# magicat777/Audio-Analyzer-OMEGA

Measured on NVIDIA B200. Metric: stream-seconds of 48 kHz stereo analysed/sec (multi-res FFT+LUFS+TP), higher is better.
Workload: dtype f32 (FFT, combine, K-weighting in a float32 delta-form state, sample peaks of the true-peak meter; its four transforms per frame pair in f16x2; tensor-core GEMM on (hi, lo) half operands with fp32 accumulators for the few-bin resolutions) + f64 (meter statistics)

## Files before the change

### audio-analyzer-omega_b200/csrc/omega4_cuda.cu

```cuda
#include "../../include/omega4_cuda.h"

#include <cuda_runtime.h>
#include <math.h>
#include <stdio.h>
#include <stdlib.h>
#include <string.h>

#include <algorithm>
#include <map>
#include <mutex>
#include <set>
#include <string>
#include <vector>

#include "bars_kernel.cuh"
#include "blockdft_kernel.cuh"
#include "blockdft_tc_kernel.cuh"
#include "fft_core.cuh"
#include "kweight_kernel.cuh"
#include "kweight32_kernel.cuh"
#include "loudness_kernel.cuh"
#include "misc_kernels.cuh"
#include "octave_kernel.cuh"
#include "multires_kernel.cuh"
// ... 22 lines not shown
    } while (0)

extern "C" const char* omega4_last_error(void) { return g_err.c_str(); }
extern "C" int omega4_abi_version(void) { return OMEGA4_ABI_VERSION; }
extern "C" int omega4_device_count(void) {
    int n = 0;
    if (cudaGetDeviceCount(&n) != cudaSuccess) { cudaGetLastError(); return 0; }
    return n;
}

static int ilog2(int n) { int l = 0; while ((1 << l) < n) ++l; return l; }
static bool is_pow2(int n) { return n > 0 && (n & (n - 1)) == 0; }

struct Twiddles { float2* twM = nullptr; float2* twN = nullptr; float2* tw4W = nullptr; };
static std::mutex g_tw_mu;
static std::map<std::pair<int, int>, Twiddles> g_tw;

static int get_twiddles(int device, int log2m, Twiddles* out) {
    std::lock_guard<std::mutex> lk(g_tw_mu);
    auto key = std::make_pair(device, log2m);
    auto it = g_tw.find(key);
    if (it != g_tw.end()) { *out = it->second; return OMEGA4_OK; }
    const int M = 1 << log2m, N = 2 * M;
    const double two_pi = 6.283185307179586476925287;
    std::vector<float2> a(M), b(M / 2 + 1), c(3 * M + 1);
    for (int e = 0; e < M; ++e) a[e] = make_float2((float)cos(two_pi * e / M), (float)-sin(two_pi * e / M));
    for (int k = 0; k <= M / 2; ++k) b[k] = make_float2((float)cos(two_pi * k / N), (float)-sin(two_pi * k / N));
    for (int j = 0; j <= 3 * M; ++j) c[j] = make_float2((float)cos(two_pi * j / (4.0 * N)), (float)sin(two_pi * j / (4.0 * N)));
    Twiddles t;
    CK(cudaMalloc(&t.twM, a.size() * sizeof(float2)));
    CK(cudaMalloc(&t.twN, b.size() * sizeof(float2)));
    CK(cudaMalloc(&t.tw4W, c.size() * sizeof(float2)));
    CK(cudaMemcpy(t.twM, a.data(), a.size() * sizeof(float2), cudaMemcpyHostToDevice));
    CK(cudaMemcpy(t.twN, b.data(), b.size() * sizeof(float2), cudaMemcpyHostToDevice));
    CK(cudaMemcpy(t.tw4W, c.data(), c.size() * sizeof(float2), cudaMemcpyHostToDevice));
    g_tw[key] = t;
    *out = t;
    return OMEGA4_OK;
}

template <int L>
static int launch_multires_t(const MultiresArgs& a, cudaStream_t s) {
    using S = FftShape<L>;
    const int fpc = a.rounds * S::CONC;
    const long long tiles = (a.n_frames + fpc - 1) / fpc;
    const long long grid = tiles * a.n_ch;
    if (grid <= 0) return OMEGA4_OK;
    if (grid > 2147483647LL) return fail(OMEGA4_ERR_INVALID, "multires grid too large");
    if constexpr (L <= 12) {
        const size_t smem = multires_local_smem_bytes<L>(a.need_cnt, a.n_tb);
        CK(cudaFuncSetAttribute(multires_local_kernel<L>, cudaFuncAttributeMaxDynamicSharedMemorySize, (int)smem));
        multires_local_kernel<L><<<(unsigned)grid, 256, smem, s>>>(a);
    } else {
        const size_t smem = multires_smem_bytes<L>(a.need_cnt);
        CK(cudaFuncSetAttribute(multires_kernel<L>, cudaFuncAttributeMaxDynamicSharedMemorySize, (int)smem));
        multires_kernel<L><<<(unsigned)grid, S::NT, smem, s>>>(a);
    }
    CK(cudaGetLastError());
    return OMEGA4_OK;
}

static int launch_multires(int log2m, const MultiresArgs& a, cudaStream_t s) {
    switch (log2m) {
        case 8: return launch_multires_t<8>(a, s);
        case 9: return launch_multires_t<9>(a, s);
        case 10: return launch_multires_t<10>(a, s);
        case 11: return launch_multires_t<11>(a, s);
        case 12: return launch_multires_t<12>(a, s);
        case 13: return launch_multires_t<13>(a, s);
        case 14: return launch_multires_t<14>(a, s);
    }
    return fail(OMEGA4_ERR_UNSUPPORTED, "fft size must be a power of two in 512 .. 32768");
}

static int default_rounds(int n_frames, int conc) {
    int r = 16;
    while (r > 1 && (long long)r * conc > n_frames) r >>= 1;
    return r;
}

static void fill_truepeak_steps(TruePeakArgs* t) {
    const double two_pi = 6.283185307179586476925287;
    for (int p = 1; p <= 3; ++p) {
        for (int j = 0; j < 16; ++j) {
            const int jj = j < 8 ? j : j - 16;
            t->step[p - 1][j] = make_float2((float)cos(two_pi * p * jj / 64.0), (float)sin(two_pi * p * jj / 64.0));
        }
        t->nyq[p - 1] = (float)cos(two_pi * p / 8.0);
    }
}

static int launch_truepeak(const TruePeakArgs& a, cudaStream_t s) {
    constexpr int L = 11;
    using S = FftShape<L>;
    const size_t smem = truepeak_smem_bytes<L>();
    CK(cudaFuncSetAttribute(truepeak_kernel<L>, cudaFuncAttributeMaxDynamicSharedMemorySize, (int)smem));
    const int ppc = a.rounds * S::CONC;
    const int n_pairs = (a.n_frames + 1) / 2;
    const long long grid = (long long)((n_pairs + ppc - 1) / ppc) * a.n_ch;
    if (grid <= 0) return OMEGA4_OK;
    if (grid > 2147483647LL) return fail(OMEGA4_ERR_INVALID, "truepeak grid too large");
    truepeak_kernel<L><<<(unsigned)grid, S::NT, smem, s>>>(a);
    CK(cudaGetLastError());
    return OMEGA4_OK;
}

static int launch_truepeak16(const TruePeakArgs& a, cudaStream_t s) {
    constexpr int L = 11;
    using S = FftShape<L>;
    const size_t smem = truepeak16_smem_bytes<L>();
    CK(cudaFuncSetAttribute(truepeak16_kernel<L>, cudaFuncAttributeMaxDynamicSharedMemorySize, (int)smem));
    const int ppc = a.rounds * S::CONC;
    const int n_pairs = (a.n_frames + 1) / 2;
    const long long grid = (long long)((n_pairs + ppc - 1) / ppc) * a.n_ch;
    if (grid <= 0) return OMEGA4_OK;
    if (grid > 2147483647LL) return fail(OMEGA4_ERR_INVALID, "truepeak grid too large");
    truepeak16_kernel<L><<<(unsigned)grid, S::NT, smem, s>>>(a);
    CK(cudaGetLastError());
    return OMEGA4_OK;
}

template <bool F64, bool WT>
static int launch_kweight_t(const KweightArgs& a, cudaStream_t s) {
    const size_t smem = kweight_smem_bytes();
    CK(cudaFuncSetAttribute(kweight_kernel<F64, WT>, cudaFuncAttributeMaxDynamicSharedMemorySize, (int)smem));
    const int fpc = a.frames_per_warp * KW_WARPS;
    const long long grid = (long long)((a.n_frames + fpc - 1) / fpc) * a.n_ch;
    if (grid <= 0) return OMEGA4_OK;
    if (grid > 2147483647LL) return fail(OMEGA4_ERR_INVALID, "kweight grid too large");
    kweight_kernel<F64, WT><<<(unsigned)grid, KW_WARPS * 32, smem, s>>>(a);
    CK(cudaGetLastError());
    return OMEGA4_OK;
}

static int launch_kweight(const KweightArgs& a, cudaStream_t s) {
    if (a.x_is_f64) return a.weighted_out ? launch_kweight_t<true, true>(a, s) : launch_kweight_t<true, false>(a, s);
    return a.weighted_out ? launch_kweight_t<false, true>(a, s) : launch_kweight_t<false, false>(a, s);
}

static int launch_kweight32(const Kweight32Args& a, cudaStream_t s) {
    const size_t smem = kweight32_smem_bytes();
    CK(cudaFuncSetAttribute(kweight32_kernel, cudaFuncAttributeMaxDynamicSharedMemorySize, (int)smem));
    const int fpc = a.frames_per_warp * KW32_WARPS;
    const long long grid = (long long)((a.n_frames + fpc - 1) / fpc) * a.n_ch;
    if (grid <= 0) return OMEGA4_OK;
    if (grid > 2147483647LL) return fail(OMEGA4_ERR_INVALID, "kweight grid too large");
    kweight32_kernel<<<(unsigned)grid, KW32_WARPS * 32, smem, s>>>(a);
    CK(cudaGetLastError());
    return OMEGA4_OK;
}

static int launch_stats(const StatsArgs& a, cudaStream_t s) {
    if (a.n_ch <= 0) return OMEGA4_OK;
    if (!a.fresh && a.n_frames == 1 && a.first_frame == 0 && !getenv("OMEGA4_STATS_WALK")) {
        stats_push1_kernel<<<a.n_ch, ST_P1_THREADS, 0, s>>>(a);
    } else if (a.fresh) {
        const size_t smem = stats_smem_bytes<false>();
        CK(cudaFuncSetAttribute(stats_kernel<false>, cudaFuncAttributeMaxDynamicSharedMemorySize, (int)smem));
        stats_kernel<false><<<a.n_ch, ST_THREADS, smem, s>>>(a);
    } else {
        const size_t smem = stats_smem_bytes<true>();
        CK(cudaFuncSetAttribute(stats_kernel<true>, cudaFuncAttributeMaxDynamicSharedMemorySize, (int)smem));
        stats_kernel<true><<<a.n_ch, ST_THREADS, smem, s>>>(a);
    }
    CK(cudaGetLastError());
    return OMEGA4_OK;
}

static int launch_s16_convert(const int16_t* in, long long stream_stride, int il, int n_streams, long long n_frames,
                              float* out, long long out_stride, cudaStream_t s) {
    if (n_streams <= 0 || n_frames <= 0) return OMEGA4_OK;
    if (n_streams > 65535) return fail(OMEGA4_ERR_INVALID, "too many streams for one int16 conversion launch (max 65535)");
    const long long per_stream = n_frames * il;
    dim3 grid((unsigned)((per_stream + 1023) / 1024), (unsigned)n_streams);
    s16_deinterleave_kernel<<<grid, 256, 0, s>>>(in, stream_stride, il, n_frames, out, out_stride);
    CK(cudaGetLastError());
    return OMEGA4_OK;
}

static void mat2_mul(const double* a, const double* b, double* c) {
    double r[4] = {a[0] * b[0] + a[1] * b[2], a[0] * b[1] + a[1] * b[3],
                   a[2] * b[0] + a[3] * b[2], a[2] * b[1] + a[3] * b[3]};
    memcpy(c, r, sizeof r);
}

static void build_biquad(const double* b, const double* a, int order, KwBiquad* q) {
    memset(q, 0, sizeof *q);
    const double a0 = a[0];
    q->b0 = b[0] / a0; q->b1 = b[1] / a0; q->b2 = order >= 2 ? b[2] / a0 : 0.0;
    q->a1 = a[1] / a0; q->a2 = order >= 2 ? a[2] / a0 : 0.0;
    q->pad = 3 * (order + 1);
    if (order >= 2) {
        double zi0, zi1;
        const double m00 = 1.0 + q->a1, m01 = -1.0, m10 = q->a2, m11 = 1.0;
        const double r0 = q->b1 - q->a1 * q->b0, r1 = q->b2 - q->a2 * q->b0;
        const double det = m00 * m11 - m01 * m10;
        zi0 = (r0 * m11 - m01 * r1) / det;
        zi1 = (m00 * r1 - m10 * r0) / det;
        q->yi0 = -zi1 / q->a2;
        q->yi1 = (-zi0 + q->a1 * zi1 / q->a2) / q->a2;
    } else {
        const double zi0 = (q->b1 - q->a1 * q->b0) / (1.0 + q->a1);
        q->yi0 = -zi0 / q->a1;
        q->yi1 = 0.0;
    }
    const double Cm[4] = {-q->a1, -q->a2, 1.0, 0.0};
    double P[4] = {Cm[0], Cm[1], Cm[2], Cm[3]};
    for (int i = 0; i < KW_L; ++i) {
        if (i < KW_SUBMAX) { q->g[i][0] = P[0]; q->g[i][1] = P[1]; }
        if (i + 1 == 16) memcpy(q->c16, P, sizeof P);
        if (i + 1 == 17) memcpy(q->c17, P, sizeof P);
        if (i + 1 < KW_L) mat2_mul(Cm, P, P);
    }
    memcpy(q->phi[0], P, sizeof P);
    for (int j = 1; j < 5; ++j) mat2_mul(q->phi[j - 1], q->phi[j - 1], q->phi[j]);
    auto inv_pow = [&](int k, double* out) {
        if (k == 0) { out[0] = 1; out[1] = 0; out[2] = 0; out[3] = 1; return; }
        if (order >= 2) {
            const double det1 = Cm[0] * Cm[3] - Cm[1] * Cm[2];
            const double Ci[4] = {Cm[3] / det1, -Cm[1] / det1, -Cm[2] / det1, Cm[0] / det1};
            double R[4] = {Ci[0], Ci[1], Ci[2], Ci[3]};
            for (int i = 1; i < k; ++i) mat2_mul(Ci, R, R);
            memcpy(out, R, sizeof R);
        } else {
            out[0] = pow(-q->a1, -(double)k); out[1] = 0; out[2] = 0; out[3] = 0;
        }
    };
    inv_pow(KW_PAD - q->pad, q->cinv_f);
    inv_pow(KW_SLACK + KW_PAD - q->pad, q->cinv_b);
}

struct ResInfo {
    int n = 0, log2m = 0, bins = 0;
    float weight = 1.f;
    float* window = nullptr;
    float* binw = nullptr;
    int n_tb = 0;
    int* tb_idx = nullptr;
    int* tb_lo = nullptr;
    float* tb_frac = nullptr;
    int need_lo = 0, need_cnt = 0;
    Twiddles tw;
};

struct SparseRes {
    int r = 0, nk = 0, nt = 0, B = 0, col0 = 0;
    bool td = false;
    int xoff = 0;
    float2* T = nullptr;
    float* kw = nullptr;
    int* tb_pos = nullptr;
};

struct SparseSet {
    int n = 0;
    SparseRes sp[OMEGA4_MAX_RES];
    int of_res[OMEGA4_MAX_RES];
    int cols = 0, qs = 0;
    float* E = nullptr;
    uint8_t* Eimg = nullptr;
    float e_inv = 1.f;
    int n_halves = 0;
    bool fusable = false;
    int nkx = 0;
    short gB[TC_MAX_GROUPS], gX[TC_MAX_GROUPS], gN[TC_MAX_GROUPS], gS[TC_MAX_GROUPS];
    SparseSet() { for (int i = 0; i < OMEGA4_MAX_RES; ++i) of_res[i] = -1; }
    void release() {
        for (int i = 0; i < OMEGA4_MAX_RES; ++i) { cudaFree(sp[i].T); cudaFree(sp[i].kw); cudaFree(sp[i].tb_pos); }
        cudaFree(E); cudaFree(Eimg);
    }
};

struct DevBuf {
    void* p = nullptr;
    size_t cap = 0;
    int ensure(size_t bytes) {
        if (bytes <= cap) return OMEGA4_OK;
        if (p) cudaFree(p);
        p = nullptr; cap = 0;
        CK(cudaMalloc(&p, bytes));
        cap = bytes;
        return OMEGA4_OK;
    }
    void release() { if (p) cudaFree(p); p = nullptr; cap = 0; }
};

struct omega4_bars {
    int device = 0, T = 0, n_valid = 0, p_lo = 0, normalize_max = 0;
    float p_frac = 0.f, scale = 0.8f;
    int* bands = nullptr; float* gain = nullptr; float* sf = nullptr; float* sfc = nullptr;
    DevBuf h_spec, h_out, h_peak, h_state, state_in;
};

static int bars_launch(omega4_bars* b, cudaStream_t s, const float* spec, int n_ch, int n_hops, float* state, int fresh,
                       float* band_values, float* peak_values, DevBuf* state_copy) {
    BarsArgs a;
    memset(&a, 0, sizeof a);
    a.T = b->T; a.n_ch = n_ch; a.n_hops = n_hops; a.n_valid = b->n_valid; a.bands = b->bands; a.gain = b->gain;
    a.sf = b->sf; a.sfc = b->sfc; a.p_lo = b->p_lo; a.p_frac = b->p_frac; a.scale = b->scale;
    a.normalize_max = b->normalize_max; a.fresh = (fresh || !state) ? 1 : 0;
    a.spec = spec; a.bars_out = band_values; a.peaks_out = peak_values; a.state = state;
    const size_t st_bytes = (size_t)n_ch * (1 + b->n_valid) * sizeof(float);
    const size_t smem = bars_smem_bytes(b->T, b->n_valid);
    if (smem > 200 * 1024) return fail(OMEGA4_ERR_UNSUPPORTED, "spectrum too long for the bars kernel");
    if (b->T > 32 * BARS_MAXV) return fail(OMEGA4_ERR_UNSUPPORTED, "spectrum too long for the bars kernel (max 1024 bins)");
    if (b->T <= 512) CK(cudaFuncSetAttribute(bars_kernel<16>, cudaFuncAttributeMaxDynamicSharedMemorySize, (int)smem));
    else CK(cudaFuncSetAttribute(bars_kernel<32>, cudaFuncAttributeMaxDynamicSharedMemorySize, (int)smem));
    a.seg = n_ch >= 1024 ? 4 * BARS_SEG : BARS_SEG;
    const long long grid = (long long)n_ch * ((n_hops + a.seg - 1) / a.seg);
    if (grid > 2147483647LL) return fail(OMEGA4_ERR_INVALID, "bars grid too large");
    if (a.state && !a.fresh && n_hops > a.seg) {
        int rc = state_copy->ensure(st_bytes); if (rc) return rc;
        CK(cudaMemcpyAsync(state_copy->p, a.state, st_bytes, cudaMemcpyDeviceToDevice, s));
        a.state_in = (const float*)state_copy->p;
    }
    if (b->T <= 512) bars_kernel<16><<<(unsigned)grid, BARS_WARPS * 32, smem, s>>>(a);
// ... 1970 lines not shown
```

### audio-analyzer-omega_b200/csrc/stats_kernel.cuh

```cuda
#pragma once
#include <cuda_runtime.h>
#include <math_constants.h>

namespace o4 {

constexpr int ST_M = 24;
constexpr int ST_S = 180;
constexpr int ST_I = 3600;
constexpr int ST_P = 60;
constexpr int ST_SORT = 4096;
constexpr int ST_THREADS = 32;
constexpr int ST_STATE = 8 + ST_I + ST_P;

struct StatsArgs {
    const double* lufs;
    const double* tp;
    int n_ch;
    int n_frames;
    int first_frame;
    double gate;
    double* state;
    float* out;
    int fresh;
};

__device__ __forceinline__ double st_percentile(const double* s, int n, double q) {
    double vi = (double)n * q + (1.0 + q * (1.0 - 1.0 - 1.0)) - 1.0;
    if (vi < 0.0) vi = 0.0;
    if (vi > (double)(n - 1)) vi = (double)(n - 1);
    double fl = floor(vi);
    int lo = (int)fl;
    int hi = lo + 1 < n ? lo + 1 : n - 1;
    double t = vi - fl;
    double av = s[lo], bv = s[hi];
    double d = bv - av;
    return (t >= 0.5) ? (bv - d * (1.0 - t)) : (av + d * t);
}

__device__ __forceinline__ int warp_lower_bound(const float* s, int n, float v, int lane) {
    int lo = 0, hi = n;
    while (lo < hi) {
        const int step = (hi - lo + 31) >> 5;
        const int idx = lo + lane * step;
        const bool less = (idx < hi) && (s[idx] < v);
        const int c = __popc(__ballot_sync(0xffffffffu, less));
        if (step == 1) return lo + c;
        if (c == 0) return lo;
        const int nhi = min(hi, lo + c * step);
        lo = lo + (c - 1) * step + 1;
        hi = nhi;
    }
    return lo;
}

__device__ __forceinline__ double st_percentile_f(const float* s, int n, double q) {
    double vi = (double)n * q + (1.0 + q * (1.0 - 1.0 - 1.0)) - 1.0;
    if (vi < 0.0) vi = 0.0;
    if (vi > (double)(n - 1)) vi = (double)(n - 1);
    const double fl = floor(vi);
    const int lo = (int)fl;
    const int hi = lo + 1 < n ? lo + 1 : n - 1;
    const double t = vi - fl;
    const double av = (double)s[lo], bv = (double)s[hi];
    const double d = bv - av;
    return (t >= 0.5) ? (bv - d * (1.0 - t)) : (av + d * t);
}

template <bool CARRIED>
constexpr int stw_smem() { return ((CARRIED ? ST_SORT : ST_I) + 64) * (int)sizeof(float); }

template <bool CARRIED>
__global__ void __launch_bounds__(32)
stats_kernel(const __grid_constant__ StatsArgs a) {
    extern __shared__ __align__(16) unsigned char smem_raw[];
    float* srt = reinterpret_cast<float*>(smem_raw);
    float* pkw = srt + (CARRIED ? ST_SORT : ST_I);

    const int ch = blockIdx.x;
    const int lane = threadIdx.x;
    double* st = a.state + (size_t)ch * ST_STATE;
    const double* lufs = a.lufs + (size_t)ch * a.n_frames;
    const double* tps = a.tp + (size_t)ch * a.n_frames;
    const float gate = (float)a.gate;

    int n_hist = 0, n_tp = 0;
    double cur[5] = {-100.0, -100.0, -100.0, 0.0, -100.0};
    if (CARRIED && !a.fresh) {
        n_hist = min(max((int)st[0], 0), ST_I);
        n_tp = min(max((int)st[1], 0), ST_P);
        if (n_hist > 0 || n_tp > 0 || st[7] != 0.0) {
#pragma unroll
            for (int i = 0; i < 5; ++i) cur[i] = st[2 + i];
        }
    }
    const int n0 = n_hist;
    const double* win0 = st + 8;
    if (CARRIED) for (int i = lane; i < n_tp; i += 32) pkw[i] = (float)st[8 + ST_I + i];
    __syncwarp();
    int pk_head = 0, ns = 0, cnt_m = 0, cnt_s = 0;
    double sum_i = 0.0, sum_m = 0.0, sum_s = 0.0, inv_m = 1.0, inv_s = 1.0, inv_ns = 0.0;
    float tp_max = -CUDART_INF_F;
    if (CARRIED && (n_hist > 0 || n_tp > 0)) {
        for (int i = lane; i < ST_SORT; i += 32) {
            float v = (i < n_hist) ? (float)win0[i] : CUDART_INF_F;
            srt[i] = (v > gate) ? v : CUDART_INF_F;
        }
        __syncwarp();
        for (int k = 2; k <= ST_SORT; k <<= 1) {
            for (int j = k >> 1; j > 0; j >>= 1) {
                for (int i = lane; i < ST_SORT; i += 32) {
                    int ixj = i ^ j;
                    if (ixj > i) {
                        float x = srt[i], y = srt[ixj];
                        bool up = ((i & k) == 0);
                        if ((x > y) == up) { srt[i] = y; srt[ixj] = x; }
                    }
                }
                __syncwarp();
            }
        }
        double si = 0.0; int c = 0;
        for (int i = lane; i < n_hist; i += 32) { float v = (float)win0[i]; if (v > gate) { ++c; si += (double)v; } }
#pragma unroll
        for (int o = 16; o > 0; o >>= 1) { c += __shfl_xor_sync(0xffffffffu, c, o); si += __shfl_xor_sync(0xffffffffu, si, o); }
        ns = c; sum_i = si;
        cnt_m = n_hist < ST_M ? n_hist : ST_M;
        cnt_s = n_hist < ST_S ? n_hist : ST_S;
        for (int i = n_hist - cnt_m; i < n_hist; ++i) sum_m += (double)(float)win0[i];
        for (int i = n_hist - cnt_s; i < n_hist; ++i) sum_s += (double)(float)win0[i];
        if (cnt_m > 0) inv_m = 1.0 / (double)cnt_m;
        if (cnt_s > 0) inv_s = 1.0 / (double)cnt_s;
        if (ns > 0) inv_ns = 1.0 / (double)ns;
        float m = -CUDART_INF_F;
        for (int i = lane; i < n_tp; i += 32) m = fmaxf(m, pkw[i]);
#pragma unroll
        for (int o = 16; o > 0; o >>= 1) m = fmaxf(m, __shfl_xor_sync(0xffffffffu, m, o));
        tp_max = m;
    }
    const int kbeg = a.first_frame < a.n_frames ? a.first_frame : a.n_frames;
    for (int k = lane; k < kbeg; k += 32) {
        float* orow = a.out + ((size_t)ch * a.n_frames + k) * 5;
#pragma unroll
        for (int i = 0; i < 5; ++i) orow[i] = (float)cur[i];
    }

    auto pushed_before = [&](int p, int D) -> float {
        const int q = p - D;
        if (q >= 0) return (float)lufs[kbeg + q];
        const int c = n0 + q;
        return (CARRIED && c >= 0) ? (float)win0[c] : 0.f;
    };
    float my_l = 0.f, my_t = 0.f, my_oi = 0.f, my_os = 0.f, my_om = 0.f;
    for (int k = kbeg; k < a.n_frames; ++k) {
        const int kk = (k - kbeg) & 31;
        if (kk == 0) {
            const int idx = k + lane;
            const bool ok = idx < a.n_frames;
            my_l = ok ? (float)lufs[idx] : 0.f;
            my_t = ok ? (float)tps[idx] : 0.f;
            my_oi = ok ? pushed_before(idx - kbeg, ST_I) : 0.f;
            my_os = ok ? pushed_before(idx - kbeg, ST_S) : 0.f;
            my_om = ok ? pushed_before(idx - kbeg, ST_M) : 0.f;
        }
        const float nv = __shfl_sync(0xffffffffu, my_l, kk);
        const float ntp = __shfl_sync(0xffffffffu, my_t, kk);
        const float ov_i = __shfl_sync(0xffffffffu, my_oi, kk);
        const float ov_s = __shfl_sync(0xffffffffu, my_os, kk);
        const float ov_m = __shfl_sync(0xffffffffu, my_om, kk);
        const bool has_old = (n_hist == ST_I);
        const float ov = has_old ? ov_i : 0.f;
        const bool rem = has_old && (ov > gate);
        const bool ins = (nv > gate);
        const int prem = rem ? warp_lower_bound(srt, ns, ov, lane) : -1;
        const int pins = ins ? warp_lower_bound(srt, ns, nv, lane) : -1;
        int lo = ns, hi = -1;
        if (prem >= 0 && pins >= 0) {
            if (pins > prem) { lo = prem + 1; hi = pins - 1; }
            else { lo = pins; hi = prem - 1; }
        } else if (prem >= 0) { lo = prem + 1; hi = ns - 1; }
        else if (pins >= 0) { lo = pins; hi = ns - 1; }
        const bool left = (prem >= 0 && (pins < 0 || pins > prem));
        if (hi >= lo) {
            constexpr int SB = 8;
            if (left) {
                for (int base = lo; base <= hi; base += 32 * SB) {
                    float tb[SB];
#pragma unroll
                    for (int j = 0; j < SB; ++j) { int idx = base + lane + 32 * j; if (idx <= hi) tb[j] = srt[idx]; }
                    __syncwarp();
#pragma unroll
                    for (int j = 0; j < SB; ++j) { int idx = base + lane + 32 * j; if (idx <= hi) srt[idx - 1] = tb[j]; }
                }
            } else {
                for (int top = hi; top >= lo; top -= 32 * SB) {
                    float tb[SB];
#pragma unroll
                    for (int j = 0; j < SB; ++j) { int idx = top - lane - 32 * j; if (idx >= lo) tb[j] = srt[idx]; }
                    __syncwarp();
#pragma unroll
                    for (int j = 0; j < SB; ++j) { int idx = top - lane - 32 * j; if (idx >= lo) srt[idx + 1] = tb[j]; }
                }
            }
        }
        __syncwarp();
        if (!has_old) ++n_hist;
        const int ns_new = ns + (ins ? 1 : 0) - (rem ? 1 : 0);
        if (rem) sum_i -= (double)ov;
        if (ins) sum_i += (double)nv;
        if (ns_new != ns) inv_ns = ns_new > 0 ? 1.0 / (double)ns_new : 0.0;
        ns = ns_new;
        if (ns == 0) sum_i = 0.0;
        sum_m += (double)nv;
        if (cnt_m == ST_M) sum_m -= (double)ov_m;
        else { ++cnt_m; inv_m = 1.0 / (double)cnt_m; }
        sum_s += (double)nv;
        if (cnt_s == ST_S) sum_s -= (double)ov_s;
        else { ++cnt_s; inv_s = 1.0 / (double)cnt_s; }
        int pslot;
        float otp = -CUDART_INF_F;
        if (n_tp == ST_P) { pslot = pk_head; otp = pkw[pk_head]; pk_head = (pk_head + 1 == ST_P) ? 0 : pk_head + 1; }
        else { pslot = n_tp; ++n_tp; }
        __syncwarp();
        if (lane == 0) {
            if (ins) srt[pins - ((prem >= 0 && pins > prem) ? 1 : 0)] = nv;
            pkw[pslot] = ntp;
        }
        __syncwarp();
        if (ntp >= tp_max) tp_max = ntp;
        else if (otp >= tp_max) {
            float m = -CUDART_INF_F;
            for (int i = lane; i < n_tp; i += 32) m = fmaxf(m, pkw[i]);
#pragma unroll
            for (int o = 16; o > 0; o >>= 1) m = fmaxf(m, __shfl_xor_sync(0xffffffffu, m, o));
            tp_max = m;
        }
        double pv = (ns > 0 && lane < 2) ? st_percentile_f(srt, ns, lane == 0 ? 0.95 : 0.10) : 0.0;
        const double p10 = __shfl_sync(0xffffffffu, pv, 1);
        cur[0] = sum_m * inv_m;
        cur[1] = sum_s * inv_s;
        cur[2] = (ns > 0) ? sum_i * inv_ns : -100.0;
        cur[3] = (ns > 0) ? __shfl_sync(0xffffffffu, pv, 0) - p10 : 0.0;
        cur[4] = (double)tp_max;
        if (lane == 0) {
            float* orow = a.out + ((size_t)ch * a.n_frames + k) * 5;
            orow[0] = (float)cur[0]; orow[1] = (float)cur[1]; orow[2] = (float)cur[2];
            orow[3] = (float)cur[3]; orow[4] = (float)cur[4];
        }
    }
    __syncwarp();
    {
        const int P = a.n_frames - kbeg;
        const int shift = n0 + P - n_hist;
        for (int b0 = 0; b0 < n_hist; b0 += 32) {
            const int i = b0 + lane;
            double v = 0.0;
            if (i < n_hist) {
                const int c = i + shift;
                v = (c < n0) ? (double)(float)win0[c] : (double)(float)lufs[kbeg + c - n0];
            }
            __syncwarp();
            if (i < n_hist) st[8 + i] = v;
        }
    }
    {
        float pv2[2] = {0.f, 0.f};
#pragma unroll
        for (int j = 0; j < 2; ++j) { const int i = lane + 32 * j; if (i < n_tp) pv2[j] = pkw[(n_tp == ST_P) ? (pk_head + i) % ST_P : i]; }
        __syncwarp();
#pragma unroll
        for (int j = 0; j < 2; ++j) { const int i = lane + 32 * j; if (i < n_tp) st[8 + ST_I + i] = (double)pv2[j]; }
    }
    if (lane == 0) {
        st[0] = (double)n_hist; st[1] = (double)n_tp; st[7] = 1.0;
        st[2] = cur[0]; st[3] = cur[1]; st[4] = cur[2]; st[5] = cur[3]; st[6] = cur[4];
    }
}


constexpr int ST_P1_THREADS = 256;

__global__ void __launch_bounds__(ST_P1_THREADS)
stats_push1_kernel(const __grid_constant__ StatsArgs a) {
    __shared__ float win[ST_I];
    __shared__ float srt[ST_SORT];
    __shared__ float pk[ST_P];
    __shared__ double red_d[ST_P1_THREADS / 32];
    __shared__ int red_i[ST_P1_THREADS / 32];
    const int ch = blockIdx.x, tid = threadIdx.x, lane = tid & 31, warp = tid >> 5;
    double* st = a.state + (size_t)ch * ST_STATE;
    const float gate = (float)a.gate;
    const int n0 = min(max((int)st[0], 0), ST_I), p0 = min(max((int)st[1], 0), ST_P);
    const float nv = (float)a.lufs[ch], ntp = (float)a.tp[ch];
    const int drop = (n0 == ST_I) ? 1 : 0, n = n0 - drop + 1;
    for (int i = tid; i < n - 1; i += ST_P1_THREADS) win[i] = (float)st[8 + i + drop];
    const int pdrop = (p0 == ST_P) ? 1 : 0, np = p0 - pdrop + 1;
    for (int i = tid; i < np - 1; i += ST_P1_THREADS) pk[i] = (float)st[8 + ST_I + i + pdrop];
    if (tid == 0) { win[n - 1] = nv; pk[np - 1] = ntp; }
    __syncthreads();
    int nsort = 32;
    while (nsort < n) nsort <<= 1;
    int c = 0;
    double si = 0.0;
    for (int i = tid; i < nsort; i += ST_P1_THREADS) {
        const float v = (i < n) ? win[i] : CUDART_INF_F;
        const bool g = v > gate && i < n;
        srt[i] = g ? v : CUDART_INF_F;
        if (g) { ++c; si += (double)v; }
    }
#pragma unroll
    for (int o = 16; o > 0; o >>= 1) { c += __shfl_xor_sync(0xffffffffu, c, o); si += __shfl_xor_sync(0xffffffffu, si, o); }
    if (lane == 0) { red_i[warp] = c; red_d[warp] = si; }
    __syncthreads();
    for (int k = 2; k <= nsort; k <<= 1)
        for (int j = k >> 1; j > 0; j >>= 1) {
            for (int i = tid; i < nsort; i += ST_P1_THREADS) {
                const int l = i ^ j;
                if (l > i) {
                    const float x = srt[i], y = srt[l];
                    if ((x > y) == ((i & k) == 0)) { srt[i] = y; srt[l] = x; }
                }
            }
            __syncthreads();
        }
    for (int i = tid; i < n; i += ST_P1_THREADS) st[8 + i] = (double)win[i];
    for (int i = tid; i < np; i += ST_P1_THREADS) st[8 + ST_I + i] = (double)pk[i];
    if (tid == 0) {
        int ns = 0;
        double sum_i = 0.0;
        for (int w = 0; w < ST_P1_THREADS / 32; ++w) { ns += red_i[w]; sum_i += red_d[w]; }
        const int cm = n < ST_M ? n : ST_M, cs = n < ST_S ? n : ST_S;
        double sum_m = 0.0, sum_s = 0.0;
        for (int i = n - cm; i < n; ++i) sum_m += (double)win[i];
        for (int i = n - cs; i < n; ++i) sum_s += (double)win[i];
        float m = -CUDART_INF_F;
        for (int i = 0; i < np; ++i) m = fmaxf(m, pk[i]);
        double cur[5];
        cur[0] = sum_m * (1.0 / (double)cm);
        cur[1] = sum_s * (1.0 / (double)cs);
        cur[2] = ns > 0 ? sum_i * (1.0 / (double)ns) : -100.0;
        cur[3] = ns > 0 ? st_percentile_f(srt, ns, 0.95) - st_percentile_f(srt, ns, 0.10) : 0.0;
        cur[4] = (double)m;
        float* orow = a.out + (size_t)ch * 5;
        for (int i = 0; i < 5; ++i) { orow[i] = (float)cur[i]; st[2 + i] = cur[i]; }
        st[0] = (double)n; st[1] = (double)np; st[7] = 1.0;
    }
}

template <bool CARRIED>
inline size_t stats_smem_bytes() { return (size_t)stw_smem<CARRIED>(); }

}
```

Before: 283,000.

## Parallelise meter statistics with 16-warp segmented rank sort and bitmap selection

Replaces the single-warp sequential sliding-window stats kernel, which did an insertion-sort shift per frame, with a 512-thread kernel. Each segment of history plus new frames is sorted once with a bitonic sort on (value, index) keys to assign ranks. Frames are then split across warps, and each warp tracks its window membership as a rank bitmap. Percentiles come from popcount select, and the running sums come from warp prefix scans. This cuts per-frame serial work but costs a large shared-memory footprint, a per-warp initial bitmap build, and a per-frame true-peak rescan of up to 60 values.

```diff
diff --git a/audio-analyzer-omega_b200/csrc/omega4_cuda.cu b/audio-analyzer-omega_b200/csrc/omega4_cuda.cu
--- a/audio-analyzer-omega_b200/csrc/omega4_cuda.cu
+++ b/audio-analyzer-omega_b200/csrc/omega4_cuda.cu
@@ -198,16 +198,12 @@
 
 static int launch_stats(const StatsArgs& a, cudaStream_t s) {
     if (a.n_ch <= 0) return OMEGA4_OK;
-    if (!a.fresh && a.n_frames == 1 && a.first_frame == 0 && !getenv("OMEGA4_STATS_WALK")) {
+    if (!a.fresh && a.n_frames == 1 && a.first_frame == 0) {
         stats_push1_kernel<<<a.n_ch, ST_P1_THREADS, 0, s>>>(a);
-    } else if (a.fresh) {
-        const size_t smem = stats_smem_bytes<false>();
-        CK(cudaFuncSetAttribute(stats_kernel<false>, cudaFuncAttributeMaxDynamicSharedMemorySize, (int)smem));
-        stats_kernel<false><<<a.n_ch, ST_THREADS, smem, s>>>(a);
     } else {
-        const size_t smem = stats_smem_bytes<true>();
-        CK(cudaFuncSetAttribute(stats_kernel<true>, cudaFuncAttributeMaxDynamicSharedMemorySize, (int)smem));
-        stats_kernel<true><<<a.n_ch, ST_THREADS, smem, s>>>(a);
+        const size_t smem = stats_smem_bytes();
+        CK(cudaFuncSetAttribute(stats_kernel, cudaFuncAttributeMaxDynamicSharedMemorySize, (int)smem));
+        stats_kernel<<<a.n_ch, ST_THREADS, smem, s>>>(a);
     }
     CK(cudaGetLastError());
     return OMEGA4_OK;
diff --git a/audio-analyzer-omega_b200/csrc/stats_kernel.cuh b/audio-analyzer-omega_b200/csrc/stats_kernel.cuh
--- a/audio-analyzer-omega_b200/csrc/stats_kernel.cuh
+++ b/audio-analyzer-omega_b200/csrc/stats_kernel.cuh
@@ -9,7 +9,6 @@
 constexpr int ST_I = 3600;
 constexpr int ST_P = 60;
 constexpr int ST_SORT = 4096;
-constexpr int ST_THREADS = 32;
 constexpr int ST_STATE = 8 + ST_I + ST_P;
 
 struct StatsArgs {
@@ -24,258 +23,290 @@
     int fresh;
 };
 
-__device__ __forceinline__ double st_percentile(const double* s, int n, double q) {
-    double vi = (double)n * q + (1.0 + q * (1.0 - 1.0 - 1.0)) - 1.0;
-    if (vi < 0.0) vi = 0.0;
-    if (vi > (double)(n - 1)) vi = (double)(n - 1);
-    double fl = floor(vi);
-    int lo = (int)fl;
-    int hi = lo + 1 < n ? lo + 1 : n - 1;
-    double t = vi - fl;
-    double av = s[lo], bv = s[hi];
-    double d = bv - av;
-    return (t >= 0.5) ? (bv - d * (1.0 - t)) : (av + d * t);
-}
-
-__device__ __forceinline__ int warp_lower_bound(const float* s, int n, float v, int lane) {
-    int lo = 0, hi = n;
-    while (lo < hi) {
-        const int step = (hi - lo + 31) >> 5;
-        const int idx = lo + lane * step;
-        const bool less = (idx < hi) && (s[idx] < v);
-        const int c = __popc(__ballot_sync(0xffffffffu, less));
-        if (step == 1) return lo + c;
-        if (c == 0) return lo;
-        const int nhi = min(hi, lo + c * step);
-        lo = lo + (c - 1) * step + 1;
-        hi = nhi;
-    }
-    return lo;
-}
-
-__device__ __forceinline__ double st_percentile_f(const float* s, int n, double q) {
+__device__ __forceinline__ void st_percentile_index(int n, double q, int& lo, int& hi, double& t) {
     double vi = (double)n * q + (1.0 + q * (1.0 - 1.0 - 1.0)) - 1.0;
     if (vi < 0.0) vi = 0.0;
     if (vi > (double)(n - 1)) vi = (double)(n - 1);
     const double fl = floor(vi);
-    const int lo = (int)fl;
-    const int hi = lo + 1 < n ? lo + 1 : n - 1;
-    const double t = vi - fl;
-    const double av = (double)s[lo], bv = (double)s[hi];
+    lo = (int)fl;
+    hi = lo + 1 < n ? lo + 1 : n - 1;
+    t = vi - fl;
+}
+
+__device__ __forceinline__ double st_percentile_value(float a, float b, double t) {
+    const double av = (double)a, bv = (double)b;
     const double d = bv - av;
     return (t >= 0.5) ? (bv - d * (1.0 - t)) : (av + d * t);
 }
 
-template <bool CARRIED>
-constexpr int stw_smem() { return ((CARRIED ? ST_SORT : ST_I) + 64) * (int)sizeof(float); }
-
-template <bool CARRIED>
-__global__ void __launch_bounds__(32)
+__device__ __forceinline__ double st_percentile_f(const float* s, int n, double q) {
+    int lo, hi;
+    double t;
+    st_percentile_index(n, q, lo, hi, t);
+    return st_percentile_value(s[lo], s[hi], t);
+}
+
+__device__ __forceinline__ unsigned st_fkey(float v) {
+    const unsigned u = __float_as_uint(v);
+    return (u & 0x80000000u) ? ~u : (u | 0x80000000u);
+}
+__device__ __forceinline__ float st_fval(unsigned k) {
+    return __uint_as_float((k & 0x80000000u) ? (k & 0x7fffffffu) : ~k);
+}
+
+__device__ __forceinline__ int st_select_bit(unsigned w, int n) {
+    int pos = 0;
+#pragma unroll
+    for (int s = 16; s > 0; s >>= 1) {
+        const int c = __popc((w >> pos) & ((1u << s) - 1u));
+        if (n >= c) { n -= c; pos += s; }
+    }
+    return pos;
+}
+
+constexpr int ST_WARPS = 16;
+constexpr int ST_THREADS = ST_WARPS * 32;
+constexpr int ST_NS = 8192;
+constexpr int ST_SEG = ST_NS - ST_I;
+constexpr int ST_WPL = ST_NS / 32 / 32;
+
+struct StatsSmem {
+    unsigned long long key[ST_NS];
+    unsigned short rank[ST_NS];
+    unsigned bits[ST_WARPS][ST_NS / 32];
+    float vsel[ST_WARPS][32 * 4];
+    double fin[5];
+    int n_gated;
+};
+
+__global__ void __launch_bounds__(ST_THREADS, 2)
 stats_kernel(const __grid_constant__ StatsArgs a) {
     extern __shared__ __align__(16) unsigned char smem_raw[];
-    float* srt = reinterpret_cast<float*>(smem_raw);
-    float* pkw = srt + (CARRIED ? ST_SORT : ST_I);
-
-    const int ch = blockIdx.x;
-    const int lane = threadIdx.x;
+    StatsSmem& sm = *reinterpret_cast<StatsSmem*>(smem_raw);
+    constexpr unsigned FULL = 0xffffffffu;
+    const int ch = blockIdx.x, tid = threadIdx.x, lane = tid & 31, warp = tid >> 5;
     double* st = a.state + (size_t)ch * ST_STATE;
     const double* lufs = a.lufs + (size_t)ch * a.n_frames;
     const double* tps = a.tp + (size_t)ch * a.n_frames;
     const float gate = (float)a.gate;
 
-    int n_hist = 0, n_tp = 0;
-    double cur[5] = {-100.0, -100.0, -100.0, 0.0, -100.0};
-    if (CARRIED && !a.fresh) {
-        n_hist = min(max((int)st[0], 0), ST_I);
-        n_tp = min(max((int)st[1], 0), ST_P);
-        if (n_hist > 0 || n_tp > 0 || st[7] != 0.0) {
-#pragma unroll
-            for (int i = 0; i < 5; ++i) cur[i] = st[2 + i];
-        }
-    }
-    const int n0 = n_hist;
+    int n0 = 0, q0 = 0;
+    bool carried_out = false;
+    if (!a.fresh) {
+        n0 = min(max((int)st[0], 0), ST_I);
+        q0 = min(max((int)st[1], 0), ST_P);
+        carried_out = n0 > 0 || q0 > 0 || st[7] != 0.0;
+    }
+    auto cur0 = [&](int i) -> double { return carried_out ? st[2 + i] : (i == 3 ? 0.0 : -100.0); };
     const double* win0 = st + 8;
-    if (CARRIED) for (int i = lane; i < n_tp; i += 32) pkw[i] = (float)st[8 + ST_I + i];
-    __syncwarp();
-    int pk_head = 0, ns = 0, cnt_m = 0, cnt_s = 0;
-    double sum_i = 0.0, sum_m = 0.0, sum_s = 0.0, inv_m = 1.0, inv_s = 1.0, inv_ns = 0.0;
-    float tp_max = -CUDART_INF_F;
-    if (CARRIED && (n_hist > 0 || n_tp > 0)) {
-        for (int i = lane; i < ST_SORT; i += 32) {
-            float v = (i < n_hist) ? (float)win0[i] : CUDART_INF_F;
-            srt[i] = (v > gate) ? v : CUDART_INF_F;
+    const double* pk0 = st + 8 + ST_I;
+    const int kbeg = max(0, min(a.first_frame, a.n_frames));
+    const int P = a.n_frames - kbeg;
+    for (int k = tid; k < kbeg; k += ST_THREADS) {
+        float* orow = a.out + ((size_t)ch * a.n_frames + k) * 5;
+#pragma unroll
+        for (int i = 0; i < 5; ++i) orow[i] = (float)cur0(i);
+    }
+    auto val = [&](int c) -> float { return c < n0 ? (float)win0[c] : (float)lufs[kbeg + c - n0]; };
+    auto peak = [&](int c) -> float { return c < q0 ? (float)pk0[c] : (float)tps[kbeg + c - q0]; };
+
+    for (int p0 = 0; p0 < P; p0 += ST_SEG) {
+        const int p1 = min(P, p0 + ST_SEG);
+        const int u0 = max(0, n0 + p0 - ST_I);
+        const int U = n0 + p1 - u0;
+        int ns2 = 32;
+        while (ns2 < U) ns2 <<= 1;
+        __syncthreads();
+        for (int i = tid; i < ns2; i += ST_THREADS) {
+            unsigned long long key = ~0ull;
+            if (i < U) {
+                const float v = val(u0 + i);
+                if (v > gate) key = ((unsigned long long)st_fkey(v) << 32) | (unsigned)i;
+                sm.rank[i] = 0xffff;
+            }
+            sm.key[i] = key;
+        }
+        __syncthreads();
+        for (int k = 2; k <= ns2; k <<= 1)
+            for (int j = k >> 1; j > 0; j >>= 1) {
+                for (int t = tid; t < (ns2 >> 1); t += ST_THREADS) {
+                    const int i = 2 * t - (t & (j - 1)), l = i + j;
+                    const unsigned long long x = sm.key[i], y = sm.key[l];
+                    if ((x > y) == ((i & k) == 0)) { sm.key[i] = y; sm.key[l] = x; }
+                }
+                __syncthreads();
+            }
+        for (int r = tid; r < ns2; r += ST_THREADS) {
+            const unsigned long long k = sm.key[r];
+            if (k != ~0ull) {
+                sm.rank[(unsigned)k] = (unsigned short)r;
+                if (r + 1 == ns2 || sm.key[r + 1] == ~0ull) sm.n_gated = r + 1;
+            } else if (r == 0) {
+                sm.n_gated = 0;
+            }
+        }
+        __syncthreads();
+        const int G = sm.n_gated;
+
+        const int per = (p1 - p0 + ST_WARPS - 1) / ST_WARPS;
+        const int hs = p0 + warp * per, he = min(p1, hs + per);
+        if (hs >= he) continue;
+        unsigned* bits = sm.bits[warp];
+        const int cs = n0 + hs;
+        const int wlo = max(0, cs - ST_I);
+        for (int wd = 0; wd < ST_NS / 32; ++wd) {
+            const int r = wd * 32 + lane;
+            bool in = false;
+            if (r < G) {
+                const int i = (int)(unsigned)sm.key[r] + u0;
+                in = i >= wlo && i < cs;
+            }
+            const unsigned w = __ballot_sync(FULL, in);
+            if (lane == 0) bits[wd] = w;
         }
         __syncwarp();
-        for (int k = 2; k <= ST_SORT; k <<= 1) {
-            for (int j = k >> 1; j > 0; j >>= 1) {
-                for (int i = lane; i < ST_SORT; i += 32) {
-                    int ixj = i ^ j;
-                    if (ixj > i) {
-                        float x = srt[i], y = srt[ixj];
-                        bool up = ((i & k) == 0);
-                        if ((x > y) == up) { srt[i] = y; srt[ixj] = x; }
+        int cnt = 0;
+#pragma unroll
+        for (int j = 0; j < ST_WPL; ++j) cnt += __popc(bits[lane * ST_WPL + j]);
+        int ns = cnt;
+        double sum_i = 0.0, sum_m = 0.0, sum_s = 0.0;
+        const int cnt_m0 = min(cs, ST_M), cnt_s0 = min(cs, ST_S);
+        for (int c = wlo + lane; c < cs; c += 32) {
+            const float v = val(c);
+            if (v > gate) sum_i += (double)v;
+            if (c >= cs - cnt_s0) sum_s += (double)v;
+            if (c >= cs - cnt_m0) sum_m += (double)v;
+        }
+#pragma unroll
+        for (int o = 16; o > 0; o >>= 1) {
+            ns += __shfl_xor_sync(FULL, ns, o);
+            sum_i += __shfl_xor_sync(FULL, sum_i, o);
+            sum_m += __shfl_xor_sync(FULL, sum_m, o);
+            sum_s += __shfl_xor_sync(FULL, sum_s, o);
+        }
+        if (ns == 0) sum_i = 0.0;
+        float* vsel = sm.vsel[warp];
+
+        for (int pb = hs; pb < he; pb += 32) {
+            const int p = pb + lane;
+            const int c = n0 + p;
+            const bool mine = p < he;
+            double d_i = 0.0, d_m = 0.0, d_s = 0.0;
+            int d_n = 0, my_r = 0xffffffff;
+            float my_tp = 0.f;
+            if (mine) {
+                const float nv = val(c);
+                d_m = (double)nv - (c >= ST_M ? (double)val(c - ST_M) : 0.0);
+                d_s = (double)nv - (c >= ST_S ? (double)val(c - ST_S) : 0.0);
+                const int rn = sm.rank[c - u0];
+                const int ro = c >= ST_I ? sm.rank[c - ST_I - u0] : 0xffff;
+                if (rn != 0xffff) { d_i += (double)nv; ++d_n; }
+                if (ro != 0xffff) { d_i -= (double)val(c - ST_I); --d_n; }
+                my_r = (rn << 16) | ro;
+                const int cp = q0 + p;
+                float m = -CUDART_INF_F;
+                for (int d = max(0, cp - (ST_P - 1)); d <= cp; ++d) m = fmaxf(m, peak(d));
+                my_tp = m;
+            }
+#pragma unroll
+            for (int o = 1; o < 32; o <<= 1) {
+                const double yi = __shfl_up_sync(FULL, d_i, o), ym = __shfl_up_sync(FULL, d_m, o);
+                const double ys = __shfl_up_sync(FULL, d_s, o);
+                const int yn = __shfl_up_sync(FULL, d_n, o);
+                if (lane >= o) { d_i += yi; d_m += ym; d_s += ys; d_n += yn; }
+            }
+            const int my_ns = ns + d_n;
+            const double my_si = sum_i + d_i, my_sm = sum_m + d_m, my_ss = sum_s + d_s;
+            int lo95 = 0, hi95 = 0, lo10 = 0, hi10 = 0;
+            double t95 = 0.0, t10 = 0.0;
+            if (mine && my_ns > 0) {
+                st_percentile_index(my_ns, 0.95, lo95, hi95, t95);
+                st_percentile_index(my_ns, 0.10, lo10, hi10, t10);
+            }
+            const int my_q95 = lo95 | (hi95 << 16), my_q10 = lo10 | (hi10 << 16);
+            const int nk = min(32, he - pb);
+            for (int kk = 0; kk < nk; ++kk) {
+                const int rr = __shfl_sync(FULL, my_r, kk);
+                const int nsk = __shfl_sync(FULL, my_ns, kk);
+                const int q95 = __shfl_sync(FULL, my_q95, kk), q10 = __shfl_sync(FULL, my_q10, kk);
+                const int rn = (rr >> 16) & 0xffff, ro = rr & 0xffff;
+                const bool ins = rn != 0xffff, rem = ro != 0xffff;
+                if (lane == 0) {
+                    if (rem) bits[ro >> 5] &= ~(1u << (ro & 31));
+                    if (ins) bits[rn >> 5] |= 1u << (rn & 31);
+                }
+                cnt += (ins && (rn >> 8) == lane ? 1 : 0) - (rem && (ro >> 8) == lane ? 1 : 0);
+                __syncwarp();
+                if (nsk > 0) {
+                    int incl = cnt;
+#pragma unroll
+                    for (int o = 1; o < 32; o <<= 1) {
+                        const int y = __shfl_up_sync(FULL, incl, o);
+                        if (lane >= o) incl += y;
                     }
-                }
-                __syncwarp();
-            }
-        }
-        double si = 0.0; int c = 0;
-        for (int i = lane; i < n_hist; i += 32) { float v = (float)win0[i]; if (v > gate) { ++c; si += (double)v; } }
-#pragma unroll
-        for (int o = 16; o > 0; o >>= 1) { c += __shfl_xor_sync(0xffffffffu, c, o); si += __shfl_xor_sync(0xffffffffu, si, o); }
-        ns = c; sum_i = si;
-        cnt_m = n_hist < ST_M ? n_hist : ST_M;
-        cnt_s = n_hist < ST_S ? n_hist : ST_S;
-        for (int i = n_hist - cnt_m; i < n_hist; ++i) sum_m += (double)(float)win0[i];
-        for (int i = n_hist - cnt_s; i < n_hist; ++i) sum_s += (double)(float)win0[i];
-        if (cnt_m > 0) inv_m = 1.0 / (double)cnt_m;
-        if (cnt_s > 0) inv_s = 1.0 / (double)cnt_s;
-        if (ns > 0) inv_ns = 1.0 / (double)ns;
-        float m = -CUDART_INF_F;
-        for (int i = lane; i < n_tp; i += 32) m = fmaxf(m, pkw[i]);
-#pragma unroll
-        for (int o = 16; o > 0; o >>= 1) m = fmaxf(m, __shfl_xor_sync(0xffffffffu, m, o));
-        tp_max = m;
-    }
-    const int kbeg = a.first_frame < a.n_frames ? a.first_frame : a.n_frames;
-    for (int k = lane; k < kbeg; k += 32) {
-        float* orow = a.out + ((size_t)ch * a.n_frames + k) * 5;
-#pragma unroll
-        for (int i = 0; i < 5; ++i) orow[i] = (float)cur[i];
-    }
-
-    auto pushed_before = [&](int p, int D) -> float {
-        const int q = p - D;
-        if (q >= 0) return (float)lufs[kbeg + q];
-        const int c = n0 + q;
-        return (CARRIED && c >= 0) ? (float)win0[c] : 0.f;
-    };
-    float my_l = 0.f, my_t = 0.f, my_oi = 0.f, my_os = 0.f, my_om = 0.f;
-    for (int k = kbeg; k < a.n_frames; ++k) {
-        const int kk = (k - kbeg) & 31;
-        if (kk == 0) {
-            const int idx = k + lane;
-            const bool ok = idx < a.n_frames;
-            my_l = ok ? (float)lufs[idx] : 0.f;
-            my_t = ok ? (float)tps[idx] : 0.f;
-            my_oi = ok ? pushed_before(idx - kbeg, ST_I) : 0.f;
-            my_os = ok ? pushed_before(idx - kbeg, ST_S) : 0.f;
-            my_om = ok ? pushed_before(idx - kbeg, ST_M) : 0.f;
-        }
-        const float nv = __shfl_sync(0xffffffffu, my_l, kk);
-        const float ntp = __shfl_sync(0xffffffffu, my_t, kk);
-        const float ov_i = __shfl_sync(0xffffffffu, my_oi, kk);
-        const float ov_s = __shfl_sync(0xffffffffu, my_os, kk);
-        const float ov_m = __shfl_sync(0xffffffffu, my_om, kk);
-        const bool has_old = (n_hist == ST_I);
-        const float ov = has_old ? ov_i : 0.f;
-        const bool rem = has_old && (ov > gate);
-        const bool ins = (nv > gate);
-        const int prem = rem ? warp_lower_bound(srt, ns, ov, lane) : -1;
-        const int pins = ins ? warp_lower_bound(srt, ns, nv, lane) : -1;
-        int lo = ns, hi = -1;
-        if (prem >= 0 && pins >= 0) {
-            if (pins > prem) { lo = prem + 1; hi = pins - 1; }
-            else { lo = pins; hi = prem - 1; }
-        } else if (prem >= 0) { lo = prem + 1; hi = ns - 1; }
-        else if (pins >= 0) { lo = pins; hi = ns - 1; }
-        const bool left = (prem >= 0 && (pins < 0 || pins > prem));
-        if (hi >= lo) {
-            constexpr int SB = 8;
-            if (left) {
-                for (int base = lo; base <= hi; base += 32 * SB) {
-                    float tb[SB];
-#pragma unroll
-                    for (int j = 0; j < SB; ++j) { int idx = base + lane + 32 * j; if (idx <= hi) tb[j] = srt[idx]; }
-                    __syncwarp();
-#pragma unroll
-                    for (int j = 0; j < SB; ++j) { int idx = base + lane + 32 * j; if (idx <= hi) srt[idx - 1] = tb[j]; }
-                }
-            } else {
-                for (int top = hi; top >= lo; top -= 32 * SB) {
-                    float tb[SB];
-#pragma unroll
-                    for (int j = 0; j < SB; ++j) { int idx = top - lane - 32 * j; if (idx >= lo) tb[j] = srt[idx]; }
-                    __syncwarp();
-#pragma unroll
-                    for (int j = 0; j < SB; ++j) { int idx = top - lane - 32 * j; if (idx >= lo) srt[idx + 1] = tb[j]; }
-                }
-            }
-        }
-        __syncwarp();
-        if (!has_old) ++n_hist;
-        const int ns_new = ns + (ins ? 1 : 0) - (rem ? 1 : 0);
-        if (rem) sum_i -= (double)ov;
-        if (ins) sum_i += (double)nv;
-        if (ns_new != ns) inv_ns = ns_new > 0 ? 1.0 / (double)ns_new : 0.0;
-        ns = ns_new;
-        if (ns == 0) sum_i = 0.0;
-        sum_m += (double)nv;
-        if (cnt_m == ST_M) sum_m -= (double)ov_m;
-        else { ++cnt_m; inv_m = 1.0 / (double)cnt_m; }
-        sum_s += (double)nv;
-        if (cnt_s == ST_S) sum_s -= (double)ov_s;
-        else { ++cnt_s; inv_s = 1.0 / (double)cnt_s; }
-        int pslot;
-        float otp = -CUDART_INF_F;
-        if (n_tp == ST_P) { pslot = pk_head; otp = pkw[pk_head]; pk_head = (pk_head + 1 == ST_P) ? 0 : pk_head + 1; }
-        else { pslot = n_tp; ++n_tp; }
-        __syncwarp();
-        if (lane == 0) {
-            if (ins) srt[pins - ((prem >= 0 && pins > prem) ? 1 : 0)] = nv;
-            pkw[pslot] = ntp;
-        }
-        __syncwarp();
-        if (ntp >= tp_max) tp_max = ntp;
-        else if (otp >= tp_max) {
-            float m = -CUDART_INF_F;
-            for (int i = lane; i < n_tp; i += 32) m = fmaxf(m, pkw[i]);
-#pragma unroll
-            for (int o = 16; o > 0; o >>= 1) m = fmaxf(m, __shfl_xor_sync(0xffffffffu, m, o));
-            tp_max = m;
-        }
-        double pv = (ns > 0 && lane < 2) ? st_percentile_f(srt, ns, lane == 0 ? 0.95 : 0.10) : 0.0;
-        const double p10 = __shfl_sync(0xffffffffu, pv, 1);
-        cur[0] = sum_m * inv_m;
-        cur[1] = sum_s * inv_s;
-        cur[2] = (ns > 0) ? sum_i * inv_ns : -100.0;
-        cur[3] = (ns > 0) ? __shfl_sync(0xffffffffu, pv, 0) - p10 : 0.0;
-        cur[4] = (double)tp_max;
-        if (lane == 0) {
-            float* orow = a.out + ((size_t)ch * a.n_frames + k) * 5;
-            orow[0] = (float)cur[0]; orow[1] = (float)cur[1]; orow[2] = (float)cur[2];
-            orow[3] = (float)cur[3]; orow[4] = (float)cur[4];
-        }
-    }
-    __syncwarp();
-    {
-        const int P = a.n_frames - kbeg;
-        const int shift = n0 + P - n_hist;
-        for (int b0 = 0; b0 < n_hist; b0 += 32) {
-            const int i = b0 + lane;
-            double v = 0.0;
-            if (i < n_hist) {
-                const int c = i + shift;
-                v = (c < n0) ? (double)(float)win0[c] : (double)(float)lufs[kbeg + c - n0];
+                    const int k0 = q95 & 0xffff, k1 = q95 >> 16, k2 = q10 & 0xffff, k3 = q10 >> 16;
+                    const unsigned b0 = __ballot_sync(FULL, incl > k0), b1 = __ballot_sync(FULL, incl > k1);
+                    const unsigned b2 = __ballot_sync(FULL, incl > k2), b3 = __ballot_sync(FULL, incl > k3);
+                    const int tk = lane == 0 ? k0 : lane == 1 ? k1 : lane == 2 ? k2 : k3;
+                    const unsigned tb = lane == 0 ? b0 : lane == 1 ? b1 : lane == 2 ? b2 : b3;
+                    const int owner = __ffs(tb) - 1;
+                    const int ex = __shfl_sync(FULL, incl - cnt, owner);
+                    if (lane < 4) {
+                        int local = tk - ex;
+                        const uint4* wp = reinterpret_cast<const uint4*>(bits + owner * ST_WPL);
+                        const uint4 A = wp[0], B = wp[1];
+                        const unsigned w[ST_WPL] = {A.x, A.y, A.z, A.w, B.x, B.y, B.z, B.w};
+                        unsigned word = 0;
+                        int wi = 0;
+                        bool found = false;
+#pragma unroll
+                        for (int j = 0; j < ST_WPL; ++j) {
+                            const int pc = __popc(w[j]);
+                            if (!found) {
+                                if (local < pc) { word = w[j]; wi = j; found = true; }
+                                else local -= pc;
+                            }
+                        }
+                        const int pos = (owner * ST_WPL + wi) * 32 + st_select_bit(word, local);
+                        vsel[kk * 4 + lane] = st_fval((unsigned)(sm.key[pos] >> 32));
+                    }
+                }
             }
             __syncwarp();
-            if (i < n_hist) st[8 + i] = v;
-        }
-    }
-    {
-        float pv2[2] = {0.f, 0.f};
-#pragma unroll
-        for (int j = 0; j < 2; ++j) { const int i = lane + 32 * j; if (i < n_tp) pv2[j] = pkw[(n_tp == ST_P) ? (pk_head + i) % ST_P : i]; }
-        __syncwarp();
-#pragma unroll
-        for (int j = 0; j < 2; ++j) { const int i = lane + 32 * j; if (i < n_tp) st[8 + ST_I + i] = (double)pv2[j]; }
-    }
-    if (lane == 0) {
-        st[0] = (double)n_hist; st[1] = (double)n_tp; st[7] = 1.0;
-        st[2] = cur[0]; st[3] = cur[1]; st[4] = cur[2]; st[5] = cur[3]; st[6] = cur[4];
-    }
-}
-
+            if (mine) {
+                const double lra = my_ns > 0 ? st_percentile_value(vsel[lane * 4 + 0], vsel[lane * 4 + 1], t95) -
+                                               st_percentile_value(vsel[lane * 4 + 2], vsel[lane * 4 + 3], t10) : 0.0;
+                const int cnt_m = min(c + 1, ST_M), cnt_s = min(c + 1, ST_S);
+                const double m = my_sm * (1.0 / (double)cnt_m), s = my_ss * (1.0 / (double)cnt_s);
+                const double i = my_ns > 0 ? my_si * (1.0 / (double)my_ns) : -100.0;
+                float* orow = a.out + ((size_t)ch * a.n_frames + kbeg + p) * 5;
+                orow[0] = (float)m; orow[1] = (float)s; orow[2] = (float)i; orow[3] = (float)lra; orow[4] = my_tp;
+                if (p == P - 1) {
+                    sm.fin[0] = m; sm.fin[1] = s; sm.fin[2] = i; sm.fin[3] = lra; sm.fin[4] = (double)my_tp;
+                }
+            }
+            __syncwarp();
+            ns = __shfl_sync(FULL, my_ns, nk - 1);
+            sum_i = __shfl_sync(FULL, my_si, nk - 1);
+            sum_m = __shfl_sync(FULL, my_sm, nk - 1);
+            sum_s = __shfl_sync(FULL, my_ss, nk - 1);
+        }
+    }
+    __syncthreads();
+    const int nh = min(n0 + P, ST_I), nq = min(q0 + P, ST_P);
+    float* stage = reinterpret_cast<float*>(sm.key);
+    for (int i = tid; i < nh; i += ST_THREADS) stage[i] = val(n0 + P - nh + i);
+    for (int i = tid; i < nq; i += ST_THREADS) stage[ST_I + i] = peak(q0 + P - nq + i);
+    __syncthreads();
+    for (int i = tid; i < nh; i += ST_THREADS) st[8 + i] = (double)stage[i];
+    for (int i = tid; i < nq; i += ST_THREADS) st[8 + ST_I + i] = (double)stage[ST_I + i];
+    if (tid == 0) {
+        st[0] = (double)nh; st[1] = (double)nq; st[7] = 1.0;
+        for (int i = 0; i < 5; ++i) st[2 + i] = P > 0 ? sm.fin[i] : cur0(i);
+    }
+}
+
+inline size_t stats_smem_bytes() { return sizeof(StatsSmem); }
 
 constexpr int ST_P1_THREADS = 256;
 
@@ -346,7 +377,4 @@
     }
 }
 
-template <bool CARRIED>
-inline size_t stats_smem_bytes() { return (size_t)stw_smem<CARRIED>(); }
-
-}
+}
```

New measurement: 290,700 (median of 6 runs). +2.7%, better.
